# parsakhaz/multimodal-image-similarity-search

Measured on AMD Instinct MI355X. Metric: images/s CLIP-B/32 encode @ bs256; Mvec/s cosine top-10 over 10M x 512, higher is better.
Workload: dtype bf16

## Files before the change

### multimodal-image-similarity-search_amd/csrc/gemm_bf16_p256.h

```cpp
#pragma once
#include <type_traits>
#include "gemm_bf16_256.h"

#define P256_BC (8 * G256_SLOT)
#define P256_TABLE (P256_BC + 4096)
#define P256_TILES (P256_TABLE + 2048)
#define P256_RAW (P256_TILES + 256)
#define P256_FTAB (P256_RAW + 16384)

__device__ __forceinline__ f16x8 p256_widen_f8(u32x2 w) {
    typedef _Float16 h2 __attribute__((ext_vector_type(2)));
    typedef float f2 __attribute__((ext_vector_type(2)));
    f16x8 r;
#pragma unroll
    for (int i = 0; i < 2; ++i) {
        const f2 lo = __builtin_amdgcn_cvt_pk_f32_fp8((int)w[i], false);
        const f2 hi = __builtin_amdgcn_cvt_pk_f32_fp8((int)w[i], true);
        const h2 l2 = __builtin_bit_cast(h2, __builtin_amdgcn_cvt_pkrtz(lo[0], lo[1]));
        const h2 g2 = __builtin_bit_cast(h2, __builtin_amdgcn_cvt_pkrtz(hi[0], hi[1]));
        r[4 * i + 0] = l2[0]; r[4 * i + 1] = l2[1]; r[4 * i + 2] = g2[0]; r[4 * i + 3] = g2[1];
    }
    return r;
}

template <int EPI, int XP>
__global__ __launch_bounds__(512, 2) void gemm256p_kernel(const __bf16* __restrict__ A, const __bf16* __restrict__ W, int M,
                                                          int N, int K, GemmEpi ep) {
    extern __shared__ __attribute__((aligned(16))) char smem[];
    typedef __bf16 IN_T;
    typedef bf16x8 frag;
    constexpr bool FOLD = (EPI == MMISS_EPI_LNFOLD_BF16 || EPI == MMISS_EPI_LNFOLD_QGELU_BF16);
    constexpr bool GELU = (EPI == MMISS_EPI_BIAS_QGELU_BF16 || EPI == MMISS_EPI_LNFOLD_QGELU_BF16);
    static_assert(FOLD == (XP > 0), "statistic pieces exist exactly in the folded modes");
    constexpr bool FINAL = FOLD && XP == 1;
    constexpr int EX = 16 + 1 + XP;
    const int tid = threadIdx.x;
    const int lane = tid & 63;
    const int wave = __builtin_amdgcn_readfirstlane(tid >> 6);
    const int wm = wave >> 2, wn = wave & 3;
    const int fr = lane & 15, fg = lane >> 4;
    const int nbm = M >> 8, nbn = N >> 8;
    const int nt = K / GEMM_BK;

    const int T = nbm * nbn, G = gridDim.x;
    const int pb = xcd_remap(blockIdx.x, G);
    const int full_rounds = T / G, rem = T - full_rounds * G;
    const bool halves = full_rounds >= 1 && rem > 0 && 2 * rem <= G;
    const int nfull = full_rounds + ((!halves && pb < rem) ? 1 : 0);
    const int nhalf = (halves && pb < 2 * rem) ? 1 : 0;
    const int mine = nfull + nhalf;
    if (tid < mine && tid < 64) {
        const bool hf = tid >= nfull;
        const int L = hf ? full_rounds * G + (pb >> 1) : tid * G + pb;
        int bm_, bn_;
        tile_order(L, nbm, nbn, ep.m_fast, bm_, bn_);
        reinterpret_cast<unsigned*>(smem + P256_TILES)[tid] = (unsigned)bm_ | ((unsigned)bn_ << 16) | (hf ? (1u << 30) : 0u) |
                                                             ((hf && (pb & 1)) ? (1u << 31) : 0u);
    }
    __syncthreads();
    auto tile_of = [&](int i, int& bm, int& bn, int& half) {
        const unsigned pk = (unsigned)__builtin_amdgcn_readfirstlane(((const __attribute__((address_space(3))) int*)(smem + P256_TILES))[i]);
        bm = pk & 0xffff;
        bn = (pk >> 16) & 0x3fff;
        half = (pk >> 30) ? 1 + (int)(pk >> 31) : 0;
    };

    const int r_in = lane >> 3, p = lane & 7;
    const int src_chunk = (p ^ r_in) * 8;
    const int a_vo = (((wave >> 2) * 128 + (wave & 3) * 16 + r_in) * K + src_chunk) * 2;
    const int w_vo = (((wave >> 1) * 64 + (wave & 1) * 16 + r_in) * K + src_chunk) * 2;
    const __amdgpu_buffer_rsrc_t srdA = __builtin_amdgcn_make_buffer_rsrc(const_cast<__bf16*>(A), 0, 0x7fffffff, 0x00020000);
    const __amdgpu_buffer_rsrc_t srdW = __builtin_amdgcn_make_buffer_rsrc(const_cast<__bf16*>(W), 0, 0x7fffffff, 0x00020000);
    const int row8 = 8 * K * 2;
    const int w_row8 = row8;
    constexpr bool W8 = false;
    const int stage_dst = wave * 2048;
#define P256_SLOT(which, b) (((which) * 2 + (b)) * G256_SLOT)
#define P256_BLDS(srd, vo, so, dst) \
    __builtin_amdgcn_raw_ptr_buffer_load_lds(srd, (__attribute__((address_space(3))) void*)(dst), 16, vo, so, 0, 0)
#define P256_BLDS4(srd, vo, so, dst) \
    __builtin_amdgcn_raw_ptr_buffer_load_lds(srd, (__attribute__((address_space(3))) void*)(dst), 4, vo, so, 0, 0)
#define P256_STAGE(which, b, oA, oW, LIVE)                                                                   \
    {                                                                                                       \
        char* dst_ = smem + P256_SLOT(which, b) + stage_dst;                                                \
        if constexpr ((which) < 2) {                                                                        \
            const int so_ = (oA);                                                                           \
            if (LIVE) {                                                                                     \
                P256_BLDS(srdA, a_vo, so_, dst_);                                                           \
                P256_BLDS(srdA, a_vo, so_ + row8, dst_ + 1024);                                             \
            } else {                                                                                        \
                P256_BLDS4(srdA, a_vo, so_, dst_);                                                          \
                P256_BLDS4(srdA, a_vo, so_ + row8, dst_ + 1024);                                            \
            }                                                                                               \
        } else if constexpr (W8) {                                                                          \
             \
            const int so_ = (oW) + ((which) & 1) * 4 * w_row8;                                              \
            char* dst8_ = smem + P256_SLOT(which, b) + wave * 1024;                                         \
            P256_BLDS(srdW, w_vo, so_, dst8_);                                                              \
        } else {                                                                                            \
            const int so_ = (oW) + ((which) & 1) * 4 * w_row8;                                              \
            P256_BLDS(srdW, w_vo, so_, dst_);                                                               \
            P256_BLDS(srdW, w_vo, so_ + w_row8, dst_ + 1024);                                               \
        }                                                                                                   \
    }
    auto stage_x = [&](int bm, int bn, int par) {
        const float* src = ((FOLD && wave >= 4) ? ep.aux : ep.bias) + bn * 256 + (wave & 3) * 64 + lane;
        __builtin_amdgcn_global_load_lds((const __attribute__((address_space(1))) void*)src,
                                         (__attribute__((address_space(3))) void*)(smem + P256_BC + par * 2048 + wave * 256), 4, 0, 0);
        if constexpr (FINAL) {
            const float* fs = ep.ln_final + (size_t)bm * 512 + wave * 64 + lane;
            __builtin_amdgcn_global_load_lds((const __attribute__((address_space(1))) void*)fs,
                                             (__attribute__((address_space(3))) void*)(smem + P256_FTAB + par * 2048 + wave * 256), 4, 0, 0);
        } else if constexpr (FOLD) {
            const char* st = reinterpret_cast<const char*>(ep.ln_stats) + (size_t)bm * 256 * (size_t)(XP * 32) + lane * 16;
#pragma unroll
            for (int q = 0; q < XP; ++q) glds16(st + (wave * XP + q) * 1024, smem + P256_RAW + (wave * XP + q) * 1024);
        }
    };

    uint32_t ab[2], wb[2];
#pragma unroll
    for (int s = 0; s < 2; ++s) {
        ab[s] = (wm * 64 + fr) * 128 + (((4 * s + fg) ^ (fr & 7)) << 4);
        wb[s] = P256_SLOT(2, 0) + (wn * 32 + fr) * 128 + (((4 * s + fg) ^ (fr & 7)) << 4);
    }
    frag am[4][2];
    frag wq[2][2][2];
    f32x4 acc[4][8];
#pragma unroll
    for (int i = 0; i < 4; ++i)
#pragma unroll
        for (int j = 0; j < 8; ++j) acc[i][j] = f32x4{0.f, 0.f, 0.f, 0.f};

#define P256_READ_A(b, mq)                                                                                   \
    _Pragma("unroll") for (int mf = 0; mf < 4; ++mf) {                                                      \
        am[mf][0] = *reinterpret_cast<const frag*>(smem + ab[0] + P256_SLOT(mq, b) + mf * 2048);            \
        am[mf][1] = *reinterpret_cast<const frag*>(smem + ab[1] + P256_SLOT(mq, b) + mf * 2048);            \
    }
#define P256_READ_W(b, nq)                                                                                   \
    if constexpr (W8) {                                                                                     \
        _Pragma("unroll") for (int nf = 0; nf < 2; ++nf) {                                                  \
            wq[nq][nf][0] = __builtin_bit_cast(frag, p256_widen_f8(*reinterpret_cast<const u32x2*>(smem + wb[0] + P256_SLOT(nq, b) + nf * 1024))); \
            wq[nq][nf][1] = __builtin_bit_cast(frag, p256_widen_f8(*reinterpret_cast<const u32x2*>(smem + wb[1] + P256_SLOT(nq, b) + nf * 1024))); \
        }                                                                                                   \
    } else {                                                                                                \
        _Pragma("unroll") for (int nf = 0; nf < 2; ++nf) {                                                  \
            wq[nq][nf][0] = *reinterpret_cast<const frag*>(smem + wb[0] + P256_SLOT(nq, b) + nf * 2048);    \
            wq[nq][nf][1] = *reinterpret_cast<const frag*>(smem + wb[1] + P256_SLOT(nq, b) + nf * 2048);    \
        }                                                                                                   \
    }
#define P256_MMA_HALF(mq, nq, s)                                                                             \
    _Pragma("unroll") for (int nf = 0; nf < 2; ++nf)                                                        \
        _Pragma("unroll") for (int mf = 0; mf < 4; ++mf)                                                    \
            acc[(nq) * 2 + nf][(mq) * 4 + mf] = MfmaIn<IN_T>::mma(                                          \
                wq[nq][nf][s], am[mf][s], acc[(nq) * 2 + nf][(mq) * 4 + mf]);
#define P256_MMA(mq, nq)                                                                                     \
    {                                                                                                       \
        __builtin_amdgcn_s_setprio(1);                                                                      \
        P256_MMA_HALF(mq, nq, 0)                                                                            \
        __builtin_amdgcn_sched_barrier(0);                                                                  \
        __builtin_amdgcn_sched_barrier(0);                                                                  \
        P256_MMA_HALF(mq, nq, 1)                                                                            \
        __builtin_amdgcn_s_setprio(0);                                                                      \
    }
#define P256_INFLIGHT 10
#define P256_WAIT(POST, WHICH)                                                                                 \
    asm volatile("s_waitcnt vmcnt(%0)" ::"n"((W8 ? ((WHICH) == 3 ? P256_INFLIGHT - 3 : P256_INFLIGHT - 2) : P256_INFLIGHT) + ((POST) ? EX : 0)) : "memory")
#define P256_BARRIER()                                                \
    {                                                                 \
        __builtin_amdgcn_sched_barrier(0);                            \
        __builtin_amdgcn_s_barrier();                                 \
        __builtin_amdgcn_sched_barrier(0);                            \
    }
#define P256_LATE_READS_DONE() \
    if (wm == 1) asm volatile("s_waitcnt lgkmcnt(0)" ::: "memory")
#define P256_KTILE(B, P0, P1, P3, FIN, HALF)                                                                       \
    {                                                                                                       \
        P256_READ_A(B, 0);                                                                                  \
        P256_READ_W(B, 0);                                                                                  \
        P256_STAGE(1, (B) ^ 1, oA1 + mA1, oW1, mA1 != 0);                                             \
        P256_LATE_READS_DONE();                                                                             \
        P256_WAIT(P0, 0);                                                  \
        P256_BARRIER();                                                                                     \
        P256_MMA(0, 0);                                                                                     \
        P256_BARRIER();                                                                                     \
        P256_READ_W(B, 1);                                                                                  \
        P256_STAGE(0, B, oA2, oW2, true);                                                   \
        P256_LATE_READS_DONE();                                                                             \
        P256_WAIT(P1, 1);                                                  \
        P256_BARRIER();                                                                                     \
        P256_MMA(0, 1);                                                                                     \
        P256_BARRIER();                                                                                     \
        if constexpr (!(HALF)) { P256_READ_A(B, 1); }                                                       \
        P256_STAGE(2, B, oA2, oW2, true);          \
        P256_LATE_READS_DONE();                                                                             \
        P256_BARRIER();                                                                                     \
        if constexpr (!(HALF)) { P256_MMA(1, 1); }                                                          \
        P256_BARRIER();                                                                                     \
        P256_STAGE(3, B, oA2, oW2, true);                                                 \
        P256_FIN_HOOK(FIN);                                                                                 \
        P256_WAIT(P3, 3);                                       \
        P256_BARRIER();                                                                                     \
        if constexpr (!(HALF)) { P256_MMA(1, 0); }                                                          \
        P256_BARRIER();                                                                                     \
        P256_ADVANCE();                                                                                     \
    }
#define P256_FIN_HOOK(FIN)                                                                                   \
    if constexpr (FOLD && !FINAL && (FIN)) {                                                                \
        if (kp == 1 && tid < 256) finalize_stats();                                                         \
    }
#define P256_ADVANCE()                                                                                       \
    oA1 = oA2; oW1 = oW2; mA1 = mA2;                                                                        \
    if (++k2 == nt) {                                                                                       \
        k2 = 0;                                                                                             \
        if (o2 + 1 < mine) ++o2;                                                                            \
        int bm_, bn_, hf_;                                                                                  \
        tile_of(o2, bm_, bn_, hf_);                                                                         \
        oA2 = bm_ * 256 * K * 2 + (hf_ == 2 ? 8 * row8 : 0);                                                \
        oW2 = bn_ * 256 * K * 2;                                                                            \
        mA2 = hf_ ? 0 : 8 * row8;                                                                           \
    } else {                                                                                                \
        oA2 += GEMM_BK * 2; oW2 += GEMM_BK * 2;                                                             \
    }

    auto finalize_stats = [&]() {
        const f32x4* st = reinterpret_cast<const f32x4*>(smem + P256_RAW + tid * (XP * 32));
        float s1 = 0.f, s2 = 0.f;
#pragma unroll
        for (int q = 0; q < XP * 2; ++q) { const f32x4 v = st[q]; s1 += v[0] + v[2]; s2 += v[1] + v[3]; }
        const float kd = (float)K;
        const float mean = s1 / kd;
        const float var = fmaxf(s2 / kd - mean * mean, 0.f);
        float* tb = reinterpret_cast<float*>(smem + P256_TABLE);
        tb[2 * tid] = mean;
        tb[2 * tid + 1] = 1.0f / sqrtf(var + ep.ln_eps);
    };

    int cbm, cbn, chalf;
    tile_of(0, cbm, cbn, chalf);
    int oA1 = cbm * 256 * K * 2 + (chalf == 2 ? 8 * row8 : 0), oW1 = cbn * 256 * K * 2;
    int oA2 = oA1 + GEMM_BK * 2, oW2 = oW1 + GEMM_BK * 2;
    int mA1 = chalf ? 0 : 8 * row8, mA2 = mA1;
    int o2 = 0, k2 = 1;
    const int dump_row = M - 1;

    stage_x(cbm, cbn, 0);
    {
        char* d0 = smem + stage_dst;
        P256_BLDS(srdA, a_vo, oA1, d0 + P256_SLOT(0, 0)); P256_BLDS(srdA, a_vo, oA1 + row8, d0 + P256_SLOT(0, 0) + 1024);
        P256_BLDS(srdW, w_vo, oW1, d0 + P256_SLOT(2, 0)); P256_BLDS(srdW, w_vo, oW1 + row8, d0 + P256_SLOT(2, 0) + 1024);
        P256_BLDS(srdW, w_vo, oW1 + 4 * row8, d0 + P256_SLOT(3, 0)); P256_BLDS(srdW, w_vo, oW1 + 5 * row8, d0 + P256_SLOT(3, 0) + 1024);
        P256_BLDS(srdA, a_vo, oA1 + mA1, d0 + P256_SLOT(1, 0)); P256_BLDS(srdA, a_vo, oA1 + mA1 + row8, d0 + P256_SLOT(1, 0) + 1024);
        P256_BLDS(srdA, a_vo, oA2, d0 + P256_SLOT(0, 1)); P256_BLDS(srdA, a_vo, oA2 + row8, d0 + P256_SLOT(0, 1) + 1024);
        P256_BLDS(srdW, w_vo, oW2, d0 + P256_SLOT(2, 1)); P256_BLDS(srdW, w_vo, oW2 + row8, d0 + P256_SLOT(2, 1) + 1024);
        P256_BLDS(srdW, w_vo, oW2 + 4 * row8, d0 + P256_SLOT(3, 1)); P256_BLDS(srdW, w_vo, oW2 + 5 * row8, d0 + P256_SLOT(3, 1) + 1024);
    }
    oA1 = oA2; oW1 = oW2;
    oA2 += GEMM_BK * 2; oW2 += GEMM_BK * 2;
    k2 = 2;
    asm volatile("s_waitcnt vmcnt(10)" ::: "memory");
    P256_BARRIER();
    if (wm == 1) P256_BARRIER();

    auto epilogue = [&](auto jn_c, int hrow, int par) {
        constexpr int JN = decltype(jn_c)::value;
        int lane_e = lane;
        asm volatile("" : "+v"(lane_e));
        const int fr = lane_e & 15, fg = lane_e >> 4;
        const char* bc = smem + P256_BC + par * 2048;
        f32x4 bias[4], cvec[4];
#pragma unroll
        for (int i = 0; i < 4; ++i) {
            bias[i] = *reinterpret_cast<const f32x4*>(bc + (wn * 64 + i * 16 + 4 * fg) * 4);
            if constexpr (FOLD) cvec[i] = *reinterpret_cast<const f32x4*>(bc + 1024 + (wn * 64 + i * 16 + 4 * fg) * 4);
        }
        float mu[JN], rs[JN];
#pragma unroll
        for (int j = 0; j < JN; ++j) {
            mu[j] = 0.f; rs[j] = 1.f;
            if constexpr (FOLD) {
                const float* tb = reinterpret_cast<const float*>(smem + (FINAL ? P256_FTAB + par * 2048 : P256_TABLE)) +
                                  2 * (wm * 128 + hrow + j * 16 + fr);
                mu[j] = tb[0]; rs[j] = tb[1];
            }
        }
        const __amdgpu_buffer_rsrc_t srdO = __builtin_amdgcn_make_buffer_rsrc(ep.out, 0, 0x7fffffff, 0x00020000);
        const int st_pol = ep.nt_out;
        char* patch = smem + P256_RAW + wave * (XP >= 2 ? XP * 1024 : 2048);
        const int rrow = lane_e >> 3, rchunk = lane_e & 7;
        const int wr_off = fr * 128, wr_sw = 2 * (fr & 7);
        const int col = cbn * 256 + wn * 64 + rchunk * 8;
#pragma unroll
        for (int j = 0; j < JN; ++j) {
#pragma unroll
            for (int i = 0; i < 4; ++i) {
                float y[4];
#pragma unroll
                for (int r = 0; r < 4; ++r) {
                    if constexpr (FOLD) y[r] = rs[j] * (acc[i][j][r] - mu[j] * cvec[i][r]) + bias[i][r];
                    else y[r] = acc[i][j][r] + bias[i][r];
                    if constexpr (GELU) y[r] = quick_gelu(y[r]);
                }
                u32x2 pk;
                pk[0] = pack_bf16x2(y[0], y[1]);
                pk[1] = pack_bf16x2(y[2], y[3]);
                *reinterpret_cast<u32x2*>(patch + wr_off + (((i * 4 + fg) ^ wr_sw) << 3)) = pk;
                acc[i][j] = f32x4{0.f, 0.f, 0.f, 0.f};
            }
            __builtin_amdgcn_fence(__ATOMIC_RELEASE, "wavefront");
            __builtin_amdgcn_wave_barrier();
            __builtin_amdgcn_fence(__ATOMIC_ACQUIRE, "wavefront");
#pragma unroll
            for (int rh = 0; rh < 2; ++rh) {
                const int row = rh * 8 + rrow;
                const u32x4 v = *reinterpret_cast<const u32x4*>(patch + row * 128 + (((2 * rchunk) ^ (2 * (row & 7))) << 3));
                const int m = cbm * 256 + wm * 128 + hrow + j * 16 + row;
                const int vo = ((m < ep.m_valid ? m : dump_row) * ep.ldo + col) * 2;
                if (st_pol == 16) __builtin_amdgcn_raw_buffer_store_b128(v, srdO, vo, 0, 16);
                else if (st_pol == 2) __builtin_amdgcn_raw_buffer_store_b128(v, srdO, vo, 0, 2);
                else __builtin_amdgcn_raw_buffer_store_b128(v, srdO, vo, 0, 0);
            }
            __builtin_amdgcn_wave_barrier();
        }
    };

    const int npair = nt >> 1;
    for (int ti = 0; ti < nfull; ++ti) {
        for (int kp = 0; kp < npair; ++kp) {
            if (kp == 0 && ti > 0) {
                P256_KTILE(0, true, true, true, false, false);
                P256_KTILE(1, true, false, false, false, false);
            } else {
                P256_KTILE(0, false, false, false, true, false);
                P256_KTILE(1, false, false, false, false, false);
            }
        }
        if (wm == 0) P256_BARRIER();
        epilogue(std::integral_constant<int, 8>{}, 0, ti & 1);
        if (ti + 1 < mine) {
            tile_of(ti + 1, cbm, cbn, chalf);
            stage_x(cbm, cbn, (ti + 1) & 1);
            if (wm == 1) P256_BARRIER();
        }
    }
    if (nhalf) {
        for (int kp = 0; kp < npair; ++kp) {
            if (kp == 0) {
                P256_KTILE(0, true, true, true, false, true);
                P256_KTILE(1, true, false, false, false, true);
            } else {
                P256_KTILE(0, false, false, false, true, true);
                P256_KTILE(1, false, false, false, false, true);
            }
        }
        if (wm == 0) P256_BARRIER();
        epilogue(std::integral_constant<int, 4>{}, chalf == 2 ? 64 : 0, nfull & 1);
    }
    asm volatile("s_waitcnt vmcnt(0)" ::: "memory");
}
#undef P256_FIN_HOOK
#undef P256_ADVANCE
#define P256_FIN_HOOK(FIN)
#define P256_ADVANCE()                                                                                       \
    oA1 = oA2; oW1 = oW2;                                                                                   \
    if (++k2 == nt) {                                                                                       \
        k2 = 0;                                                                                             \
        if (o2 + 1 < mine) ++o2;                                                                            \
        oA2 = 0; oW2 = o2 * 256 * K * WELT;                                                                 \
    } else {                                                                                                \
        oA2 += GEMM_BK * (int)sizeof(IN); oW2 += GEMM_BK * WELT;                                            \
    }

template <typename IN, int FILTER, bool W8 = false>
__global__ __launch_bounds__(512, 2) void gemm256s_kernel(const IN* __restrict__ A, const void* __restrict__ Wv, int M, int N, int K,
                                                          int strip, GemmEpi ep, StripFilter flt) {
    extern __shared__ __attribute__((aligned(16))) char smem[];
    typedef IN IN_T;
    typedef typename MfmaIn<IN>::frag frag;
    static_assert(!W8 || std::is_same<IN, _Float16>::value, "fp8 rows are widened to f16");
    constexpr int WELT = W8 ? 1 : (int)sizeof(IN);
    constexpr float WSCALE = W8 ? 1.0f / 128.0f : 1.0f;
    constexpr bool FOLD = false;
    constexpr int EX = W8 ? 1 : 0;
    const int tid = threadIdx.x;
    const int lane = tid & 63;
    const int wave = __builtin_amdgcn_readfirstlane(tid >> 6);
    const int wm = wave >> 2, wn = wave & 3;
    const int fr = lane & 15, fg = lane >> 4;
    const int nbm = M >> 8, nbn = N >> 8;
    const int nt = K / GEMM_BK;
    const int bn_begin = FILTER != 0 ? flt.bn_begin : 0;
    const int nstrips = (nbn - bn_begin + strip - 1) / strip;
    const int wg = xcd_remap(blockIdx.x, nbm * nstrips);
    const int sidx = wg / nbm, bm = wg - sidx * nbm;
    const int bn0 = bn_begin + sidx * strip;
    const int mine = (nbn - bn0 < strip) ? nbn - bn0 : strip;
    const IN* Ab = A + (size_t)bm * 256 * K;
    const char* Wb = reinterpret_cast<const char*>(Wv) + (size_t)bn0 * 256 * K * WELT;

    const int r_in = lane >> 3, p = lane & 7;
    const int src_chunk = (p ^ r_in) * 8;
    const int a_vo = (((wave >> 2) * 128 + (wave & 3) * 16 + r_in) * K + src_chunk) * (int)sizeof(IN);
    const int r8 = lane >> 2;
    const int w_vo = W8 ? (((wave >> 1) * 64 + (wave & 1) * 16 + r8) * K + (((lane & 3) ^ ((r8 >> 2) & 3)) << 4))
                        : (((wave >> 1) * 64 + (wave & 1) * 16 + r_in) * K + src_chunk) * (int)sizeof(IN);
    const __amdgpu_buffer_rsrc_t srdA = __builtin_amdgcn_make_buffer_rsrc(const_cast<IN*>(Ab), 0, 0x7fffffff, 0x00020000);
    const __amdgpu_buffer_rsrc_t srdW = __builtin_amdgcn_make_buffer_rsrc(const_cast<char*>(Wb), 0, 0x7fffffff, 0x00020000);
    const int row8 = 8 * K * (int)sizeof(IN);
    const int w_row8 = 8 * K * WELT;
    const int stage_dst = wave * 2048;
    const int mA1 = 8 * row8;
    uint32_t ab[2], wb[2];
#pragma unroll
    for (int s = 0; s < 2; ++s) {
        ab[s] = (wm * 64 + fr) * 128 + (((4 * s + fg) ^ (fr & 7)) << 4);
        wb[s] = W8 ? P256_SLOT(2, 0) + (wn * 32 + fr) * 64 + (((4 * s + fg) ^ (2 * ((fr >> 2) & 3))) << 3)
                   : P256_SLOT(2, 0) + (wn * 32 + fr) * 128 + (((4 * s + fg) ^ (fr & 7)) << 4);
    }
    frag am[4][2];
    frag wq[2][2][2];
    f32x4 acc[4][8];
#pragma unroll
    for (int i = 0; i < 4; ++i)
#pragma unroll
        for (int j = 0; j < 8; ++j) acc[i][j] = f32x4{0.f, 0.f, 0.f, 0.f};

    float tau_r[8];
#pragma unroll
    for (int j = 0; j < 8; ++j) tau_r[j] = INFINITY;
    if constexpr (FILTER != 0) {
#pragma unroll
        for (int j = 0; j < 8; ++j) {
            const int m = bm * 256 + wm * 128 + j * 16 + fr;
            if (m < ep.m_valid) tau_r[j] = flt.tau[(size_t)m * flt.tau_stride];
        }
        asm volatile("s_waitcnt vmcnt(0)" ::: "memory");
#pragma unroll
        for (int j = 0; j < 8; ++j) asm volatile("" : "+v"(tau_r[j]));
    }

    int oA1 = 0, oW1 = 0, oA2 = GEMM_BK * (int)sizeof(IN), oW2 = GEMM_BK * WELT;
    int o2 = 0, k2 = 1;
    auto stage_inv = [&](int ti_) {
        if constexpr (W8) {
            const float* src = ep.aux + (size_t)(bn0 + ti_) * 256 + wn * 64 + lane;
            __builtin_amdgcn_global_load_lds((const __attribute__((address_space(1))) void*)src,
                                             (__attribute__((address_space(3))) void*)(smem + G256_LDS + wave * 256), 4, 0, 0);
        }
    };
    {
        char* d0 = smem + stage_dst;
#define P256_PRO_W(which, b, oW)                                                                                      \
        if constexpr (W8) {                                                                                          \
            P256_BLDS(srdW, w_vo, (oW) + ((which) & 1) * 4 * w_row8, smem + P256_SLOT(which, b) + wave * 1024);      \
        } else {                                                                                                     \
            P256_BLDS(srdW, w_vo, (oW) + ((which) & 1) * 4 * w_row8, d0 + P256_SLOT(which, b));                      \
            P256_BLDS(srdW, w_vo, (oW) + ((which) & 1) * 4 * w_row8 + w_row8, d0 + P256_SLOT(which, b) + 1024);      \
        }
        P256_BLDS(srdA, a_vo, oA1, d0 + P256_SLOT(0, 0)); P256_BLDS(srdA, a_vo, oA1 + row8, d0 + P256_SLOT(0, 0) + 1024);
        P256_PRO_W(2, 0, oW1)
        P256_PRO_W(3, 0, oW1)
        P256_BLDS(srdA, a_vo, oA1 + mA1, d0 + P256_SLOT(1, 0)); P256_BLDS(srdA, a_vo, oA1 + mA1 + row8, d0 + P256_SLOT(1, 0) + 1024);
        P256_BLDS(srdA, a_vo, oA2, d0 + P256_SLOT(0, 1)); P256_BLDS(srdA, a_vo, oA2 + row8, d0 + P256_SLOT(0, 1) + 1024);
        P256_PRO_W(2, 1, oW2)
        P256_PRO_W(3, 1, oW2)
#undef P256_PRO_W
    }
    oA1 = oA2; oW1 = oW2;
    oA2 += GEMM_BK * (int)sizeof(IN); oW2 += GEMM_BK * WELT;
    k2 = 2;
    if constexpr (W8) asm volatile("s_waitcnt vmcnt(7)" ::: "memory");
    else asm volatile("s_waitcnt vmcnt(10)" ::: "memory");
    P256_BARRIER();
    if (wm == 1) P256_BARRIER();

    const int npair = nt >> 1;
    float* out = reinterpret_cast<float*>(ep.out);
    for (int ti = 0; ti < mine; ++ti) {
        for (int kp = 0; kp < npair; ++kp) {
            stage_inv(ti);
            P256_KTILE(0, W8, W8, W8, false, false);
            P256_KTILE(1, W8, false, false, false, false);
        }
        const int bn = bn0 + ti;
        const int g = (bn * 4 + wn) * 4 + fg;
        const int n0 = bn * 256 + wn * 64 + 4 * fg;
        const bool whole = (bn + 1) * 256 <= ep.p0;
        asm volatile("s_nop 11" ::: "memory");
        __builtin_amdgcn_sched_barrier(0);
        if constexpr (W8) {
            const char* ivp = smem + G256_LDS + wave * 256 + fg * 16;
#pragma unroll
            for (int i = 0; i < 4; ++i) {
                const f32x4 iv = *reinterpret_cast<const f32x4*>(ivp + i * 64);
#pragma unroll
                for (int j = 0; j < 8; ++j) acc[i][j] = acc[i][j] * iv;
            }
        }
        if constexpr (FILTER == 2) {
            uint32_t pmask[8];
            int pos[8];
#pragma unroll
            for (int j = 0; j < 8; ++j) {
                const int m = bm * 256 + wm * 128 + j * 16 + fr;
                float mx = mm_max3(acc[0][j][0], acc[0][j][1], acc[0][j][2]);
                mx = mm_max3(mx, acc[0][j][3], acc[1][j][0]);
#pragma unroll
                for (int i = 1; i < 4; ++i) {
                    mx = mm_max3(mx, acc[i][j][1], acc[i][j][2]);
                    mx = i < 3 ? mm_max3(mx, acc[i][j][3], acc[i + 1][j][0]) : mm_max2(mx, acc[i][j][3]);
                }
                mx *= WSCALE;
                uint32_t pm = 0;
                if (mx >= tau_r[j]) {
#pragma unroll
                    for (int i = 0; i < 4; ++i)
#pragma unroll
                        for (int r = 0; r < 4; ++r)
                            pm |= (acc[i][j][r] * WSCALE >= tau_r[j] && (whole || n0 + i * 16 + r < ep.p0)) ? (1u << (i * 4 + r)) : 0u;
                }
                pmask[j] = pm;
                pos[j] = 0;
                if (pm) pos[j] = atomicAdd(flt.cnt + m, __popc(pm));
#pragma unroll
                for (int i = 0; i < 4; ++i) acc[i][j] = f32x4{0.f, 0.f, 0.f, 0.f};
            }
#pragma unroll
            for (int j = 0; j < 8; ++j) {
                uint32_t pm = pmask[j];
                if (pm) {
                    const int m = bm * 256 + wm * 128 + j * 16 + fr;
                    int p = pos[j];
                    while (pm) {
                        const int b = __ffs(pm) - 1;
                        pm &= pm - 1;
                        if (p < flt.cap) flt.buf_g[(size_t)m * flt.cap + p] = n0 + (b >> 2) * 16 + (b & 3);
                        ++p;
                    }
                }
            }
            continue;
        }
#pragma unroll
        for (int j = 0; j < 8; ++j) {
            float mx = -INFINITY;
            if (whole) {
                mx = mm_max3(acc[0][j][0], acc[0][j][1], acc[0][j][2]);
                mx = mm_max3(mx, acc[0][j][3], acc[1][j][0]);
#pragma unroll
                for (int i = 1; i < 4; ++i) {
                    mx = mm_max3(mx, acc[i][j][1], acc[i][j][2]);
                    mx = i < 3 ? mm_max3(mx, acc[i][j][3], acc[i + 1][j][0]) : mm_max2(mx, acc[i][j][3]);
                }
#pragma unroll
                for (int i = 0; i < 4; ++i) acc[i][j] = f32x4{0.f, 0.f, 0.f, 0.f};
            } else {
#pragma unroll
                for (int i = 0; i < 4; ++i)
#pragma unroll
                    for (int r = 0; r < 4; ++r) {
                        const float v = (n0 + i * 16 + r < ep.p0) ? acc[i][j][r] : -INFINITY;
                        mx = fmaxf(mx, v);
                        acc[i][j][r] = 0.f;
                    }
            }
            const int m = bm * 256 + wm * 128 + j * 16 + fr;
            mx *= WSCALE;
            if constexpr (FILTER == 1) {
                int pos_ = -1;
                if (mx >= tau_r[j] && mx > -INFINITY)
                    pos_ = atomicAdd(flt.cnt + m, 1);
                acc[0][j][0] = mx;
                acc[0][j][1] = __int_as_float(pos_);
            } else {
                if (m < ep.m_valid) out[(size_t)m * ep.ldo + g] = mx;
            }
        }
        if constexpr (FILTER == 1) {
#pragma unroll
            for (int j = 0; j < 8; ++j) {
                const int m = bm * 256 + wm * 128 + j * 16 + fr;
                const int pos_ = __float_as_int(acc[0][j][1]);
                if (pos_ >= 0 && pos_ < flt.cap) {
                    flt.buf_s[(size_t)m * flt.cap + pos_] = acc[0][j][0];
                    flt.buf_g[(size_t)m * flt.cap + pos_] = g;
                }
                acc[0][j][0] = 0.f;
                acc[0][j][1] = 0.f;
            }
        }
    }
    if (wm == 0) P256_BARRIER();
    asm volatile("s_waitcnt vmcnt(0)" ::: "memory");
}

#undef P256_STAGE
#undef P256_INFLIGHT
#undef P256_MMA_HALF
#undef P256_SLOT
#undef P256_BLDS
#undef P256_BLDS4
#undef P256_READ_A
#undef P256_READ_W
#undef P256_MMA
#undef P256_WAIT
#undef P256_BARRIER
#undef P256_KTILE
#undef P256_FIN_HOOK
#undef P256_ADVANCE
#undef P256_LATE_READS_DONE

template <int EPI, int XP>
static int launch_gemm256p_inst(hipStream_t st, const void* A, const void* W, const GemmEpi& ep_in, int M, int N, int K) {
    GemmEpi ep = ep_in;
    if (ep.m_fast == 0) ep.m_fast = mmiss_option("gemm_p256_band", 8);
    ep.nt_out = mmiss_option("gemm_p256_store", 0);
    const int lds = XP == 1 ? P256_FTAB + 4096 : P256_RAW + (XP >= 2 ? XP * 8192 : 16384);
    const int T = (M / 256) * (N / 256);
    const int grid = T >= 256 ? 256 : T;
    MM_TRY(mmiss_ensure_dyn_lds(reinterpret_cast<const void*>(&gemm256p_kernel<EPI, XP>), lds));
    hipLaunchKernelGGL((gemm256p_kernel<EPI, XP>), dim3(grid), dim3(512), lds, st, reinterpret_cast<const __bf16*>(A),
                       reinterpret_cast<const __bf16*>(W), M, N, K, ep);
    MM_HIP(hipGetLastError());
    return MMISS_OK;
}

static inline bool gemm256p_ok(int epi, int M, int N, int K, bool final_stats = false) {
    if (M <= 0 || (M % 256) || N <= 0 || (N % 256) || K < 256 || (K % 256)) return false;
    if ((int64_t)(M / 256) * (N / 256) > 48 * 256 || M / 256 > 0xffff) return false;
    if ((int64_t)M * N * 2 >= (1LL << 31) || (int64_t)M * K * 2 >= (1LL << 31) || (int64_t)N * K * 2 >= (1LL << 31)) return false;
    if (epi == MMISS_EPI_LNFOLD_BF16 || epi == MMISS_EPI_LNFOLD_QGELU_BF16) return final_stats || K == 512 || K == 768;
    return epi == MMISS_EPI_BIAS_BF16 || epi == MMISS_EPI_BIAS_QGELU_BF16;
}

static int launch_gemm256p(hipStream_t st, int epi, const void* A, const void* W, const GemmEpi& ep, int M, int N, int K) {
    const bool fold = epi == MMISS_EPI_LNFOLD_BF16 || epi == MMISS_EPI_LNFOLD_QGELU_BF16;
    const bool fin = fold && ep.ln_final != nullptr;
    if (!gemm256p_ok(epi, M, N, K, fin)) MM_FAIL(MMISS_ERR_UNSUPPORTED, "gemm256p: epi=%d M=%d N=%d K=%d", epi, M, N, K);
    if (!ep.out || !ep.bias || (fold && (!ep.aux || (!fin && (!ep.ln_stats || ep.ln_parts * 64 != K)))))
        MM_FAIL(MMISS_ERR_ARG, "gemm256p: missing operand (fold=%d parts=%d)", (int)fold, ep.ln_parts);
    static const char* names[] = {"", "gemm_bf16_bias_p256", "gemm_bf16_bias_qgelu_p256"};
    const int mv = ep.m_valid < M ? ep.m_valid : M;
    const double bytes = 2.0 * ((double)mv * K + (double)N * K) + 2.0 * (double)mv * N;
    MM_PROF(fold ? (epi == MMISS_EPI_LNFOLD_BF16 ? "gemm_bf16_lnfold_bias_p256" : "gemm_bf16_lnfold_qgelu_p256") : names[epi], st,
            gemm_flops(mv, N, K), bytes);
    switch (epi) {
        case MMISS_EPI_BIAS_BF16: return launch_gemm256p_inst<MMISS_EPI_BIAS_BF16, 0>(st, A, W, ep, M, N, K);
        case MMISS_EPI_BIAS_QGELU_BF16: return launch_gemm256p_inst<MMISS_EPI_BIAS_QGELU_BF16, 0>(st, A, W, ep, M, N, K);
        case MMISS_EPI_LNFOLD_BF16:
            if (fin) return launch_gemm256p_inst<MMISS_EPI_LNFOLD_BF16, 1>(st, A, W, ep, M, N, K);
            return K == 768 ? launch_gemm256p_inst<MMISS_EPI_LNFOLD_BF16, 3>(st, A, W, ep, M, N, K)
                            : launch_gemm256p_inst<MMISS_EPI_LNFOLD_BF16, 2>(st, A, W, ep, M, N, K);
        default:
            if (fin) return launch_gemm256p_inst<MMISS_EPI_LNFOLD_QGELU_BF16, 1>(st, A, W, ep, M, N, K);
            return K == 768 ? launch_gemm256p_inst<MMISS_EPI_LNFOLD_QGELU_BF16, 3>(st, A, W, ep, M, N, K)
                            : launch_gemm256p_inst<MMISS_EPI_LNFOLD_QGELU_BF16, 2>(st, A, W, ep, M, N, K);
    }
}

template <typename IN, bool W8 = false>
static int launch_gemm256s(hipStream_t st, const void* A, const void* W, const GemmEpi& ep, int M, int N, int K, int strip,
                           const StripFilter* flt = nullptr) {
    if (M <= 0 || N <= 0 || K < 256 || (M % 256) || (N % 256) || (K % 128) || strip < 1 || strip > 32 ||
        (int64_t)strip * 256 * K * (int64_t)sizeof(IN) >= (1LL << 31) || (int64_t)256 * K * (int64_t)sizeof(IN) >= (1LL << 31))
        MM_FAIL(MMISS_ERR_UNSUPPORTED, "gemm256s: M=%d N=%d K=%d strip=%d", M, N, K, strip);
    const int nbn = N / 256;
    if (W8 && !ep.aux) MM_FAIL(MMISS_ERR_ARG, "gemm256s: fp8 rows need their inverse norms (ep.aux)");
    const int lds = G256_LDS + (W8 ? 2048 : 0);
    if (flt && (flt->bn_begin < 0 || flt->bn_begin >= nbn || !flt->tau || !flt->cnt || !flt->buf_g || flt->cap <= 0))
        MM_FAIL(MMISS_ERR_ARG, "gemm256s: bad filter");
    const int nwg = (M / 256) * ((nbn - (flt ? flt->bn_begin : 0) + strip - 1) / strip);
    auto launch = [&](auto filter_c) -> int {
        constexpr int FILTER = decltype(filter_c)::value;
        MM_TRY(mmiss_ensure_dyn_lds(reinterpret_cast<const void*>(&gemm256s_kernel<IN, FILTER, W8>), lds));
        hipLaunchKernelGGL((gemm256s_kernel<IN, FILTER, W8>), dim3(nwg), dim3(512), lds, st, reinterpret_cast<const IN*>(A),
                           W, M, N, K, strip, ep, flt ? *flt : StripFilter{});
        return MMISS_OK;
    };
    if (!flt) MM_TRY(launch(std::integral_constant<int, 0>{}));
    else if (flt->buf_s) MM_TRY(launch(std::integral_constant<int, 1>{}));
    else MM_TRY(launch(std::integral_constant<int, 2>{}));
    MM_HIP(hipGetLastError());
    return MMISS_OK;
}
```

Before: 94080.

## Interleave persistent GEMM epilogue blocks into next tile's k-loop

Splits the output epilogue of the persistent 256x256 bf16 GEMM into two-row-block pieces and slots them between MMA phases of the next tile's first and last k-pairs, so stores overlap with compute instead of stalling all waves after each tile. The next tile's staging moves into the k-loop as well, and the vmcnt wait counts are re-derived to cover the interleaved epilogue stores. This adds scheduling complexity and register pressure, since the previous tile's accumulators must stay live into the next tile, and depends on hand-tuned waitcnt arithmetic being correct.

```diff
diff --git a/multimodal-image-similarity-search_amd/csrc/gemm_bf16_p256.h b/multimodal-image-similarity-search_amd/csrc/gemm_bf16_p256.h
--- a/multimodal-image-similarity-search_amd/csrc/gemm_bf16_p256.h
+++ b/multimodal-image-similarity-search_amd/csrc/gemm_bf16_p256.h
@@ -33,7 +33,7 @@
     constexpr bool GELU = (EPI == MMISS_EPI_BIAS_QGELU_BF16 || EPI == MMISS_EPI_LNFOLD_QGELU_BF16);
     static_assert(FOLD == (XP > 0), "statistic pieces exist exactly in the folded modes");
     constexpr bool FINAL = FOLD && XP == 1;
-    constexpr int EX = 16 + 1 + XP;
+    constexpr int EPB = 2 * 2, EXO = 1 + XP;
     const int tid = threadIdx.x;
     const int lane = tid & 63;
     const int wave = __builtin_amdgcn_readfirstlane(tid >> 6);
@@ -165,7 +165,10 @@
     }
 #define P256_INFLIGHT 10
 #define P256_WAIT(POST, WHICH)                                                                                 \
-    asm volatile("s_waitcnt vmcnt(%0)" ::"n"((W8 ? ((WHICH) == 3 ? P256_INFLIGHT - 3 : P256_INFLIGHT - 2) : P256_INFLIGHT) + ((POST) ? EX : 0)) : "memory")
+    asm volatile("s_waitcnt vmcnt(%0)" ::"n"((W8 ? ((WHICH) == 3 ? P256_INFLIGHT - 3 : P256_INFLIGHT - 2) : P256_INFLIGHT) + (POST)) : "memory")
+#define P256_WAITX(C, X, WHICH)                                                                             \
+    if (C) P256_WAIT(X, WHICH);       \
+    else P256_WAIT(0, WHICH)
 #define P256_BARRIER()                                                \
     {                                                                 \
         __builtin_amdgcn_sched_barrier(0);                            \
@@ -174,32 +177,38 @@
     }
 #define P256_LATE_READS_DONE() \
     if (wm == 1) asm volatile("s_waitcnt lgkmcnt(0)" ::: "memory")
-#define P256_KTILE(B, P0, P1, P3, FIN, HALF)                                                                       \
+#define P256_KTILE(B, P0, P1, P3, FIN, HALF) P256_KTILE_E(B, P0, EX, P1, EX, P3, EX, FIN, HALF, 0, false)
+#define P256_KTILE_E(B, C0, X0, C1, X1, C3, X3, FIN, HALF, EPI, CE)                                         \
     {                                                                                                       \
+        P256_EPI_HOOK(EPI, CE, 1, 4);                             \
         P256_READ_A(B, 0);                                                                                  \
         P256_READ_W(B, 0);                                                                                  \
         P256_STAGE(1, (B) ^ 1, oA1 + mA1, oW1, mA1 != 0);                                             \
         P256_LATE_READS_DONE();                                                                             \
-        P256_WAIT(P0, 0);                                                  \
+        P256_WAITX(C0, X0, 0);                                             \
         P256_BARRIER();                                                                                     \
         P256_MMA(0, 0);                                                                                     \
         P256_BARRIER();                                                                                     \
+        P256_EPI_HOOK(EPI, CE, 1, 6);                            \
+        P256_NEXT_HOOK(EPI, CE);                      \
         P256_READ_W(B, 1);                                                                                  \
         P256_STAGE(0, B, oA2, oW2, true);                                                   \
         P256_LATE_READS_DONE();                                                                             \
-        P256_WAIT(P1, 1);                                                  \
+        P256_WAITX(C1, X1, 1);                                             \
         P256_BARRIER();                                                                                     \
         P256_MMA(0, 1);                                                                                     \
         P256_BARRIER();                                                                                     \
+        P256_EPI_HOOK(EPI, CE, 2, 0);        \
         if constexpr (!(HALF)) { P256_READ_A(B, 1); }                                                       \
         P256_STAGE(2, B, oA2, oW2, true);          \
         P256_LATE_READS_DONE();                                                                             \
         P256_BARRIER();                                                                                     \
         if constexpr (!(HALF)) { P256_MMA(1, 1); }                                                          \
         P256_BARRIER();                                                                                     \
+        P256_EPI_HOOK(EPI, CE, 2, 2);                                     \
         P256_STAGE(3, B, oA2, oW2, true);                                                 \
         P256_FIN_HOOK(FIN);                                                                                 \
-        P256_WAIT(P3, 3);                                       \
+        P256_WAITX(C3, X3, 3);                                  \
         P256_BARRIER();                                                                                     \
         if constexpr (!(HALF)) { P256_MMA(1, 0); }                                                          \
         P256_BARRIER();                                                                                     \
@@ -208,6 +217,16 @@
 #define P256_FIN_HOOK(FIN)                                                                                   \
     if constexpr (FOLD && !FINAL && (FIN)) {                                                                \
         if (kp == 1 && tid < 256) finalize_stats();                                                         \
+    }
+#define P256_EPI_HOOK(EPI, CE, FORM, J0)                                                                    \
+    if constexpr ((EPI) == (FORM)) if (CE) {                                                                \
+        if constexpr ((FORM) == 1) epi_blocks(std::integral_constant<int, J0>{}, 0, (ti - 1) & 1);          \
+        else epi_blocks(std::integral_constant<int, J0>{}, chalf == 2 ? 64 : 0, ti & 1);                    \
+    }
+#define P256_NEXT_HOOK(EPI, CE)                                                                             \
+    if constexpr ((EPI) == 1) if (CE) {                                                                     \
+        tile_of(ti, cbm, cbn, chalf);                                                                       \
+        stage_x(cbm, cbn, ti & 1);                                                                          \
     }
 #define P256_ADVANCE()                                                                                       \
     oA1 = oA2; oW1 = oW2; mA1 = mA2;                                                                        \
@@ -262,8 +281,8 @@
     P256_BARRIER();
     if (wm == 1) P256_BARRIER();
 
-    auto epilogue = [&](auto jn_c, int hrow, int par) {
-        constexpr int JN = decltype(jn_c)::value;
+    auto epi_blocks = [&](auto j0_c, int hrow, int par) {
+        constexpr int J0 = decltype(j0_c)::value;
         int lane_e = lane;
         asm volatile("" : "+v"(lane_e));
         const int fr = lane_e & 15, fg = lane_e >> 4;
@@ -274,14 +293,14 @@
             bias[i] = *reinterpret_cast<const f32x4*>(bc + (wn * 64 + i * 16 + 4 * fg) * 4);
             if constexpr (FOLD) cvec[i] = *reinterpret_cast<const f32x4*>(bc + 1024 + (wn * 64 + i * 16 + 4 * fg) * 4);
         }
-        float mu[JN], rs[JN];
-#pragma unroll
-        for (int j = 0; j < JN; ++j) {
-            mu[j] = 0.f; rs[j] = 1.f;
+        float mu[2], rs[2];
+#pragma unroll
+        for (int jj = 0; jj < 2; ++jj) {
+            mu[jj] = 0.f; rs[jj] = 1.f;
             if constexpr (FOLD) {
                 const float* tb = reinterpret_cast<const float*>(smem + (FINAL ? P256_FTAB + par * 2048 : P256_TABLE)) +
-                                  2 * (wm * 128 + hrow + j * 16 + fr);
-                mu[j] = tb[0]; rs[j] = tb[1];
+                                  2 * (wm * 128 + hrow + (J0 + jj) * 16 + fr);
+                mu[jj] = tb[0]; rs[jj] = tb[1];
             }
         }
         const __amdgpu_buffer_rsrc_t srdO = __builtin_amdgcn_make_buffer_rsrc(ep.out, 0, 0x7fffffff, 0x00020000);
@@ -291,13 +310,14 @@
         const int wr_off = fr * 128, wr_sw = 2 * (fr & 7);
         const int col = cbn * 256 + wn * 64 + rchunk * 8;
 #pragma unroll
-        for (int j = 0; j < JN; ++j) {
+        for (int jj = 0; jj < 2; ++jj) {
+            const int j = J0 + jj;
 #pragma unroll
             for (int i = 0; i < 4; ++i) {
                 float y[4];
 #pragma unroll
                 for (int r = 0; r < 4; ++r) {
-                    if constexpr (FOLD) y[r] = rs[j] * (acc[i][j][r] - mu[j] * cvec[i][r]) + bias[i][r];
+                    if constexpr (FOLD) y[r] = rs[jj] * (acc[i][j][r] - mu[jj] * cvec[i][r]) + bias[i][r];
                     else y[r] = acc[i][j][r] + bias[i][r];
                     if constexpr (GELU) y[r] = quick_gelu(y[r]);
                 }
@@ -324,43 +344,42 @@
         }
     };
 
+    constexpr int XL3 = 2 * EPB;
+    constexpr int XA0 = 3 * EPB;
+    constexpr int XA1 = 4 * EPB + EXO;
+    constexpr int XA3 = 3 * EPB + EXO;
+    constexpr int XB0 = 2 * EPB + EXO;
+    constexpr int XB1 = EPB + EXO;
     const int npair = nt >> 1;
+#define P256_PAIR(HALF)                                                                                      \
+    P256_KTILE_E(0, first, XA0, first, XA1, first, XA3, true, HALF, 1, first);                              \
+    P256_KTILE_E(1, first, XB0, first, XB1, last, XL3, false, HALF, 2, last);
     for (int ti = 0; ti < nfull; ++ti) {
         for (int kp = 0; kp < npair; ++kp) {
-            if (kp == 0 && ti > 0) {
-                P256_KTILE(0, true, true, true, false, false);
-                P256_KTILE(1, true, false, false, false, false);
-            } else {
-                P256_KTILE(0, false, false, false, true, false);
-                P256_KTILE(1, false, false, false, false, false);
-            }
-        }
-        if (wm == 0) P256_BARRIER();
-        epilogue(std::integral_constant<int, 8>{}, 0, ti & 1);
-        if (ti + 1 < mine) {
-            tile_of(ti + 1, cbm, cbn, chalf);
-            stage_x(cbm, cbn, (ti + 1) & 1);
-            if (wm == 1) P256_BARRIER();
+            const bool first = kp == 0 && ti > 0, last = kp == npair - 1;
+            P256_PAIR(false);
         }
     }
     if (nhalf) {
+        const int ti = nfull;
         for (int kp = 0; kp < npair; ++kp) {
-            if (kp == 0) {
-                P256_KTILE(0, true, true, true, false, true);
-                P256_KTILE(1, true, false, false, false, true);
-            } else {
-                P256_KTILE(0, false, false, false, true, true);
-                P256_KTILE(1, false, false, false, false, true);
-            }
-        }
-        if (wm == 0) P256_BARRIER();
-        epilogue(std::integral_constant<int, 4>{}, chalf == 2 ? 64 : 0, nfull & 1);
-    }
+            const bool first = kp == 0, last = kp == npair - 1;
+            P256_PAIR(true);
+        }
+    } else {
+        epi_blocks(std::integral_constant<int, 4>{}, 0, (nfull - 1) & 1);
+        epi_blocks(std::integral_constant<int, 6>{}, 0, (nfull - 1) & 1);
+    }
+    if (wm == 0) P256_BARRIER();
     asm volatile("s_waitcnt vmcnt(0)" ::: "memory");
 }
 #undef P256_FIN_HOOK
+#undef P256_EPI_HOOK
+#undef P256_NEXT_HOOK
 #undef P256_ADVANCE
 #define P256_FIN_HOOK(FIN)
+#define P256_EPI_HOOK(EPI, CE, FORM, J0)
+#define P256_NEXT_HOOK(EPI, CE)
 #define P256_ADVANCE()                                                                                       \
     oA1 = oA2; oW1 = oW2;                                                                                   \
     if (++k2 == nt) {                                                                                       \
@@ -604,9 +623,14 @@
 #undef P256_READ_W
 #undef P256_MMA
 #undef P256_WAIT
+#undef P256_WAITX
 #undef P256_BARRIER
 #undef P256_KTILE
+#undef P256_KTILE_E
+#undef P256_PAIR
 #undef P256_FIN_HOOK
+#undef P256_EPI_HOOK
+#undef P256_NEXT_HOOK
 #undef P256_ADVANCE
 #undef P256_LATE_READS_DONE
 
```

Result: slower. 89410 (-5.0%).
